# invictus717/MiCo

Measured on AMD Instinct MI355X. Metric: omni-modal samples/sec (ViT-g/14 fwd+bwd), higher is better.
Workload: dtype fp16

## Files before the change

### mico_amd/csrc/attention.hip

```cpp
#include "common.h"
#include <type_traits>

namespace {

constexpr float NEG_BIG = -1.0e30f;

#ifndef MICO_ATTN_PRIO
#define MICO_ATTN_PRIO 0
#endif

#ifdef MICO_ATTN_PHASES
__device__ unsigned long long g_attn_phase[4096 * 8];
#define PH_DECL unsigned long long ph_t = __builtin_readcyclecounter(), ph_acc[8] = {0, 0, 0, 0, 0, 0, 0, 0}
#define PH(slot) do { const unsigned long long n_ = __builtin_readcyclecounter(); ph_acc[slot] += n_ - ph_t; ph_t = n_; } while (0)
#define PH_STORE do { const int wg_ = (blockIdx.z * gridDim.y + blockIdx.y) * gridDim.x + blockIdx.x; \
        if (lane == 0 && wave == 0 && wg_ < 4096) for (int e_ = 0; e_ < 8; ++e_) g_attn_phase[wg_ * 8 + e_] = ph_acc[e_]; } while (0)
#else
#define PH_DECL
#define PH(slot)
#define PH_STORE
#endif

template <int HDP> struct Cfg {
    static constexpr int RS = 256;
// ... 53 lines not shown
}
template <int HDP, int KM = 0>
__device__ __forceinline__ s16x8 lds_row_frag(LDS_AS const char* tile, int r0, int ks, int lane) {
    const int row = r0 + (lane & 15), ch = ks * 4 + (lane >> 4);
    return *(LDS_AS const s16x8*)(tile + row * Cfg<HDP>::RS + ((ch ^ swz_key<KM>(row)) << 4));
}
template <int HDP, int KM = 0>
__device__ __forceinline__ s16x8 lds_tr_frag(LDS_AS const char* tile, int td, int s2, int lane) {
    const int g = lane >> 4, p = lane & 15;
    const int ch = td * 2 + ((p >> 1) & 1), half = (p & 1) * 8;
    const int r_lo = (2 * s2) * 16 + g * 4 + (p >> 2);
    const int col_b = ((ch ^ swz_key<KM>(r_lo)) << 4) + half;
    s16x4 lo = __builtin_amdgcn_ds_read_tr16_b64_v4i16((LDS_AS s16x4*)(tile + r_lo * Cfg<HDP>::RS + col_b));
    s16x4 hi = __builtin_amdgcn_ds_read_tr16_b64_v4i16((LDS_AS s16x4*)(tile + (r_lo + 16) * Cfg<HDP>::RS + col_b));
    s16x8 r;
    r[0] = lo[0]; r[1] = lo[1]; r[2] = lo[2]; r[3] = lo[3];
    r[4] = hi[0]; r[5] = hi[1]; r[6] = hi[2]; r[7] = hi[3];
    return r;
}

__device__ __forceinline__ void lds_dma16(__amdgpu_buffer_rsrc_t rsrc, unsigned lds_dst, unsigned voffset) {
    unsigned keep;
    const unsigned dst = __builtin_amdgcn_readfirstlane(lds_dst);
    asm volatile("s_mov_b32 %0, m0\n\ts_mov_b32 m0, %2\n\ts_nop 0\n\tbuffer_load_dwordx4 %1, %3, 0 offen lds\n\ts_mov_b32 m0, %0"
                 : "=&s"(keep) : "v"(voffset), "s"(dst), "s"(rsrc) : "memory");
}

__device__ __forceinline__ void* uniform_ptr(const void* ptr) {
    const unsigned long long v = (unsigned long long)ptr;
    const unsigned lo = __builtin_amdgcn_readfirstlane((unsigned)v), hi = __builtin_amdgcn_readfirstlane((unsigned)(v >> 32));
    return (void*)(((unsigned long long)hi << 32) | lo);
}

template <typename T>
__device__ __forceinline__ s16x8 pack_pair(const f32x4& a, const f32x4& b) {
    typename T16<T>::v8 v;
    v[0] = (T)a[0]; v[1] = (T)a[1]; v[2] = (T)a[2]; v[3] = (T)a[3];
    v[4] = (T)b[0]; v[5] = (T)b[1]; v[6] = (T)b[2]; v[7] = (T)b[3];
    return __builtin_bit_cast(s16x8, v);
}

__device__ __forceinline__ float group_max(float v) { return xor32_max(xor16_max(v)); }
__device__ __forceinline__ float group_sum(float v) { return xor32_sum(xor16_sum(v)); }

__device__ __forceinline__ float mask_val(const float* mask, int mode, int b, int i, int j, int Sq, int Sk) {
    if (mode == 1) return mask[(int64_t)b * Sk + j];
    if (mode == 2) return mask[((int64_t)b * Sq + i) * Sk + j];
    return 0.f;
}

template <typename T, int HDP, bool DROP, int RB, int NW = 4>
__global__ __launch_bounds__(NW * 64, 2) void attn_fwd_kernel(const T* __restrict__ q, const T* __restrict__ k,
                                                              const T* __restrict__ v, T* __restrict__ o,
                                                              float* __restrict__ lse, const mico_attn_params p) {
    using C = Cfg<HDP>;
    __shared__ __attribute__((aligned(16))) char smem[2 * C::TILE];
    LDS_AS char* kt = (LDS_AS char*)smem;
    LDS_AS char* vt = kt + C::TILE;
    const int tid = threadIdx.x, lane = tid & 63, wave = tid >> 6;
    const bool stager = NW == 4 || tid < 256;
    const int b = blockIdx.z, h = blockIdx.y, q0 = blockIdx.x * (NW * 16 * RB);
    const T* qb = q + (int64_t)b * p.q_bs + h * p.hd;
    const int kvb = p.kv_index ? p.kv_index[b] : (p.kv_batch_mod > 0 ? b % p.kv_batch_mod : b);
    const T* kb = k + (int64_t)kvb * p.k_bs + h * p.hd;
    const T* vb = v + (int64_t)kvb * p.v_bs + h * p.hd;
    const int i0 = q0 + wave * (16 * RB) + (lane & 15);
    const int g = lane >> 4;
    const bool wave_live = q0 + wave * (16 * RB) < p.Sq;

    s16x8 qf[RB][C::KS];
    f32x4 oacc[RB][C::TD];
    float m_run[RB], l_run[RB];
#pragma unroll
    for (int rb = 0; rb < RB; ++rb) {
        row_frags<T, HDP>(qf[rb], qb, p.q_rs, i0 + rb * 16, p.Sq, p.hd, lane);
#pragma unroll
        for (int t = 0; t < C::TD; ++t) oacc[rb][t] = (f32x4){0.f, 0.f, 0.f, 0.f};
        m_run[rb] = NEG_BIG;
        l_run[rb] = 0.f;
    }
    const float sc2 = p.scale * 1.4426950408889634f;

    const int nt = (p.Sk + 63) / 64;
    const TileMap<HDP> tm_a = tile_map<HDP>(p.k_rs, p.hd, tid), tm_b = tile_map<HDP>(p.v_rs, p.hd, tid);
    s16x8 kr[C::NCH], vr[C::NCH];
    if (stager) {
        tile_fetch<T, HDP>(kr, kb, p.k_rs, 0, p.Sk, tm_a);
        tile_fetch<T, HDP>(vr, vb, p.v_rs, 0, p.Sk, tm_b);
    }
    PH_DECL;
    for (int t = 0; t < nt; ++t) {
        __syncthreads();
        PH(0);
        if (stager) {
            tile_commit<HDP>(kr, kt, tm_a);
            tile_commit<HDP>(vr, vt, tm_b);
        }
        PH(1);
        __syncthreads();
        PH(2);
        if (stager && t + 1 < nt) {
            tile_fetch<T, HDP>(kr, kb, p.k_rs, (t + 1) * 64, p.Sk, tm_a);
            tile_fetch<T, HDP>(vr, vb, p.v_rs, (t + 1) * 64, p.Sk, tm_b);
        }
        PH(3);
        const bool edge = (t == nt - 1) && (p.Sk & 63);
        const int ntn = edge ? ((p.Sk - t * 64 + 15) >> 4) : 4;
        f32x4 s[RB][4];
#pragma unroll
        for (int tn = 0; tn < 4; ++tn) {
#pragma unroll
            for (int rb = 0; rb < RB; ++rb) s[rb][tn] = (f32x4){0.f, 0.f, 0.f, 0.f};
            if (tn < ntn && wave_live) {
#pragma unroll
                for (int ks = 0; ks < C::KS; ++ks) {
                    const s16x8 a = lds_row_frag<HDP>(kt, tn * 16, ks, lane);
#pragma unroll
                    for (int rb = 0; rb < RB; ++rb) s[rb][tn] = T16<T>::mfma(a, qf[rb][ks], s[rb][tn]);
                }
            }
        }
        s16x8 pf[RB][2];
        PH(4);
#pragma unroll
        for (int rb = 0; rb < RB; ++rb) {
            const int i = i0 + rb * 16;
            float mloc = NEG_BIG;
            if (!p.mask_mode && !edge) {
#pragma unroll
                for (int tn = 0; tn < 4; ++tn) {
                    s[rb][tn] *= sc2;
                    mloc = fmaxf(fmaxf(mloc, fmaxf(s[rb][tn][0], s[rb][tn][1])), fmaxf(s[rb][tn][2], s[rb][tn][3]));
                }
            } else {
#pragma unroll
                for (int tn = 0; tn < 4; ++tn)
#pragma unroll
                    for (int r = 0; r < 4; ++r) {
                        const int j = t * 64 + tn * 16 + g * 4 + r;
                        float x = s[rb][tn][r] * sc2;
                        if (j < p.Sk) {
                            if (p.mask_mode && i < p.Sq) x += mask_val(p.mask, p.mask_mode, b, i, j, p.Sq, p.Sk) * 1.4426950408889634f;
                        } else {
                            x = NEG_BIG;
                        }
                        s[rb][tn][r] = x;
                        mloc = fmaxf(mloc, x);
                    }
            }
// ... 11 lines not shown
            if (DROP) {
                const unsigned thr = drop_threshold(p.drop_p);
                const float ik = 1.f / (1.f - p.drop_p);
                const unsigned long long rowbase = (((unsigned long long)(b + p.batch0) * p.H + h) * p.Sq + i) * (unsigned long long)p.Sk;
                if ((unsigned long long)(p.B + p.batch0) * p.H * p.Sq * p.Sk <= 0xFFFFFFFFull) {
                    const unsigned h0 = p.drop_seed ^ ((unsigned)p.drop_site * 0x9E3779B9u);
                    const unsigned tb = ((unsigned)rowbase + (unsigned)(t * 64 + g * 4)) * 0x85EBCA6Bu;
#pragma unroll
                    for (int tn = 0; tn < 4; ++tn)
#pragma unroll
                        for (int r = 0; r < 4; ++r)
                            s[rb][tn][r] *= drop_hash_t(h0, tb + (unsigned)(tn * 16 + r) * 0x85EBCA6Bu) >= thr ? ik : 0.f;
                } else {
#pragma unroll
                    for (int tn = 0; tn < 4; ++tn)
#pragma unroll
                        for (int r = 0; r < 4; ++r)
                            s[rb][tn][r] *= drop_mult(p.drop_seed, p.drop_site, rowbase + (t * 64 + tn * 16 + g * 4 + r), thr, ik);
                }
            }
            l_run[rb] = l_run[rb] * alpha + group_sum(lloc);
            m_run[rb] = m_new;
#pragma unroll
            for (int t2 = 0; t2 < C::TD; ++t2) oacc[rb][t2] *= alpha;
            pf[rb][0] = pack_pair<T>(s[rb][0], s[rb][1]);
            pf[rb][1] = pack_pair<T>(s[rb][2], s[rb][3]);
        }
        PH(5);
#pragma unroll
        for (int s2 = 0; s2 < 2; ++s2) {
            if (2 * s2 >= ntn || !wave_live) continue;
#pragma unroll
            for (int td = 0; td < C::TD; ++td) {
                const s16x8 a = lds_tr_frag<HDP>(vt, td, s2, lane);
#pragma unroll
                for (int rb = 0; rb < RB; ++rb) oacc[rb][td] = T16<T>::mfma(a, pf[rb][s2], oacc[rb][td]);
            }
        }
        PH(6);
    }
    PH_STORE;
#pragma unroll
    for (int rb = 0; rb < RB; ++rb) {
        const int i = i0 + rb * 16;
        if (i < p.Sq) {
            const float inv = 1.f / l_run[rb];
            T* ob = o + (int64_t)b * p.o_bs + (int64_t)i * p.o_rs + h * p.hd;
#pragma unroll
            for (int td = 0; td < C::TD; ++td) {
                const int d = td * 16 + g * 4;
                if (d < p.hd)
                    *(s16x4*)(ob + d) = pack4<T>(oacc[rb][td][0] * inv, oacc[rb][td][1] * inv, oacc[rb][td][2] * inv, oacc[rb][td][3] * inv);
            }
            if (g == 0) lse[((int64_t)b * p.H + h) * p.Sq + i] = (m_run[rb] + __log2f(l_run[rb])) * 0.6931471805599453f;
        }
    }
}

constexpr int RES_KR = 288;

template <typename T, int HDP, int RB, int NSUB, bool ALL>
__device__ __forceinline__ void res_tile_step(LDS_AS const char* ktile, LDS_AS const char* vtile, const int key0, const int lo,
                                              const int hi, const int mode, const s16x8 (&qf)[RB][Cfg<HDP>::KS],
                                              f32x4 (&oacc)[RB][Cfg<HDP>::TD], float (&m_run)[RB], float (&l_run)[RB],
                                              const int Sk, const float sc2, const int lane,
                                              const int (&rf)[Cfg<HDP>::KS], const int (&tf)[Cfg<HDP>::TD]) {
    using C = Cfg<HDP>;
    constexpr int NH = (NSUB + 1) / 2;
    const int g = lane >> 4;
    f32x4 s[RB][NH * 2];
    if (ALL) {
        s16x8 an[C::KS];
#pragma unroll
// ... 1529 lines not shown
        }
        if (lane < 24) {
            LDS_AS float* pw = part + wave * 2 * HDP + lane * 4;
#pragma unroll
            for (int e = 0; e < 4; ++e) { pw[e] = dkx[e]; pw[HDP + e] = dvx[e]; }
        }
        asm volatile("s_waitcnt lgkmcnt(0)" ::: "memory");
        __builtin_amdgcn_s_barrier();
        if (tid < 2 * HDP / 4) {
            const int which = tid / (HDP / 4), d = (tid - which * (HDP / 4)) * 4;
            f32x4 acc = {0.f, 0.f, 0.f, 0.f};
            for (int w = 0; w < 8; ++w) {
                LDS_AS const float* prow = part + w * 2 * HDP + which * HDP + d;
                acc[0] += prow[0]; acc[1] += prow[1]; acc[2] += prow[2]; acc[3] += prow[3];
            }
            if (d < p.hd) {
                T* out = (which ? dv + (int64_t)b * p.v_bs + (int64_t)256 * p.v_rs : dk + (int64_t)b * p.k_bs + (int64_t)256 * p.k_rs) + h * p.hd + d;
                *(s16x4*)out = pack4<T>(acc[0], acc[1], acc[2], acc[3]);
            }
        }
    }
}

#endif
struct SqCfg {
    static constexpr int QMAX = 80, QR = 96;
    static constexpr int RS = 128;
    static constexpr int QT = QR * RS;
    static constexpr int KT = 32 * RS, DST = 32 * 256, WAVE = KT + DST;
    static constexpr int STAT = 2 * QR * 4;
    static constexpr int LDS = 2 * QT + STAT + 4 * WAVE;
};

__device__ __forceinline__ int sq_off(int row, int ch) { return row * SqCfg::RS + ((ch ^ ((((row >> 1) & 3) << 1) | ((row >> 3) & 1))) << 4); }
__device__ __forceinline__ s16x8 sq_row_frag(LDS_AS const char* tile, int r0, int ks, int lane) {
    return *(LDS_AS const s16x8*)(tile + sq_off(r0 + (lane & 15), ks * 4 + (lane >> 4)));
}
__device__ __forceinline__ s16x8 sq_tr_frag(LDS_AS const char* tile, int td, int s2, int lane) {
    const int g = lane >> 4, p = lane & 15;
    const int r_lo = (2 * s2) * 16 + g * 4 + (p >> 2);
    const int off = sq_off(r_lo, td * 2 + ((p >> 1) & 1)) + (p & 1) * 8;
    s16x4 lo = __builtin_amdgcn_ds_read_tr16_b64_v4i16((LDS_AS s16x4*)(tile + off));
    s16x4 hi = __builtin_amdgcn_ds_read_tr16_b64_v4i16((LDS_AS s16x4*)(tile + off + 16 * SqCfg::RS));
    s16x8 r;
    r[0] = lo[0]; r[1] = lo[1]; r[2] = lo[2]; r[3] = lo[3];
    r[4] = hi[0]; r[5] = hi[1]; r[6] = hi[2]; r[7] = hi[3];
    return r;
}

template <typename T, bool DROP, int MASK>
__global__ __launch_bounds__(256, 2) void attn_bwd_smallq_kernel(const T* __restrict__ q, const T* __restrict__ k, const T* __restrict__ v,
                                                                 const T* __restrict__ o, const T* __restrict__ d_o, const float* __restrict__ lse,
                                                                 T* __restrict__ dq, T* __restrict__ dk, T* __restrict__ dv, const mico_attn_params p) {
    using S = SqCfg;
    constexpr int HD = 64;
    __shared__ __attribute__((aligned(16))) char smem[S::LDS];
    LDS_AS char* qt = (LDS_AS char*)smem;
    LDS_AS char* dot = qt + S::QT;
    LDS_AS float* lse_t = (LDS_AS float*)(dot + S::QT);
    LDS_AS float* del_t = lse_t + S::QR;
    LDS_AS char* strips = (LDS_AS char*)smem + 2 * S::QT + S::STAT;
    const int tid = threadIdx.x, lane = tid & 63, wave = __builtin_amdgcn_readfirstlane(tid >> 6), g = lane >> 4;
    const int b = blockIdx.y, h = blockIdx.x;
    LDS_AS char* kt = strips + wave * S::WAVE;
    LDS_AS char* dst = kt + S::KT;
    const T* qb = q + (int64_t)b * p.q_bs + h * HD;
    const int kvb = p.kv_batch_mod > 0 ? b % p.kv_batch_mod : b;
    const T* kb = k + (int64_t)kvb * p.k_bs + h * HD;
    const T* vb = v + (int64_t)kvb * p.v_bs + h * HD;
    const T* ob = o + (int64_t)b * p.o_bs + h * HD;
    const T* dob = d_o + (int64_t)b * p.o_bs + h * HD;
    const int64_t stat_base = ((int64_t)b * p.H + h) * p.Sq;
    constexpr float LOG2E = 1.4426950408889634f;
    const float sc2 = p.scale * LOG2E;
    const int nstrips = (p.Sk + 31) >> 5, nrounds = (nstrips + 3) >> 2;

    s16x8 kf[2][2], vf[2][2];
#pragma unroll
    for (int kbk = 0; kbk < 2; ++kbk) {
        row_frags<T, HD>(kf[kbk], kb, p.k_rs, wave * 32 + kbk * 16 + (lane & 15), p.Sk, HD, lane);
        row_frags<T, HD>(vf[kbk], vb, p.v_rs, wave * 32 + kbk * 16 + (lane & 15), p.Sk, HD, lane);
    }
#pragma unroll
    for (int it = 0; it < 3; ++it) {
        const int c = it * 256 + tid, row = c >> 3, ch = c & 7;
        s16x8 qv = {0, 0, 0, 0, 0, 0, 0, 0}, dv8 = qv, ov = qv;
        if (row < p.Sq) {
            qv = *(const s16x8*)(qb + (int64_t)row * p.q_rs + ch * 8);
            dv8 = *(const s16x8*)(dob + (int64_t)row * p.o_rs + ch * 8);
            ov = *(const s16x8*)(ob + (int64_t)row * p.o_rs + ch * 8);
        }
        *(LDS_AS s16x8*)(qt + sq_off(row, ch)) = qv;
        *(LDS_AS s16x8*)(dot + sq_off(row, ch)) = dv8;
        float a[8], c8[8], dl = 0.f;
        unpack8<T>(ov, a);
        unpack8<T>(dv8, c8);
#pragma unroll
        for (int e = 0; e < 8; ++e) dl += a[e] * c8[e];
        dl += __shfl_xor(dl, 1);
        dl += __shfl_xor(dl, 2);
        dl += __shfl_xor(dl, 4);
        if (ch == 0) {
            del_t[row] = dl * p.scale;
            lse_t[row] = row < p.Sq ? lse[stat_base + row] * LOG2E : 0.f;
        }
    }
    __syncthreads();

    f32x4 dqw[4], dq4 = {0.f, 0.f, 0.f, 0.f};
#pragma unroll
    for (int td = 0; td < 4; ++td) dqw[td] = (f32x4){0.f, 0.f, 0.f, 0.f};

    const int nti = (p.Sq + 15) >> 4;
    const unsigned ibase = (unsigned)((((unsigned long long)(b + p.batch0) * p.H + h) * p.Sq) * (unsigned long long)p.Sk);
    const unsigned h0 = p.drop_seed ^ ((unsigned)p.drop_site * 0x9E3779B9u), tstep = (unsigned)p.Sk * 0x85EBCA6Bu;
    const unsigned thr = drop_threshold(p.drop_p);
    const float inv_keep = 1.f / (1.f - p.drop_p);
    const f32x4 zero4 = {0.f, 0.f, 0.f, 0.f};

    for (int rd = 0; rd < nrounds; ++rd) {
        const int k0 = (rd * 4 + wave) * 32;
        s16x8 nkf[2][2], nvf[2][2];
        if (rd + 1 < nrounds) {
#pragma unroll
            for (int kbk = 0; kbk < 2; ++kbk) {
                row_frags<T, HD>(nkf[kbk], kb, p.k_rs, k0 + 128 + kbk * 16 + (lane & 15), p.Sk, HD, lane);
                row_frags<T, HD>(nvf[kbk], vb, p.v_rs, k0 + 128 + kbk * 16 + (lane & 15), p.Sk, HD, lane);
            }
        }
        if (k0 < p.Sk) {
#pragma unroll
            for (int kbk = 0; kbk < 2; ++kbk)
#pragma unroll
                for (int ks = 0; ks < 2; ++ks) *(LDS_AS s16x8*)(kt + sq_off(kbk * 16 + (lane & 15), ks * 4 + g)) = kf[kbk][ks];
#pragma unroll
            for (int kbk = 0; kbk < 2; ++kbk) {
                __builtin_amdgcn_sched_barrier(0);
                const int j = k0 + kbk * 16 + (lane & 15);
                const bool jv = j < p.Sk;
                const int jc = jv ? j : p.Sk - 1;
                T* const dkb = dk + (int64_t)b * p.k_bs + (int64_t)jc * p.k_rs + h * HD;
                T* const dvb = dv + (int64_t)b * p.v_bs + (int64_t)jc * p.v_rs + h * HD;
                s16x4 okd[4], ovd[4];
                if (MASK == 0 && p.dkv_accumulate == 1) {
#pragma unroll
                    for (int td = 0; td < 4; ++td) {
                        okd[td] = *(const s16x4*)(dkb + td * 16 + g * 4);
                        ovd[td] = *(const s16x4*)(dvb + td * 16 + g * 4);
                    }
                }
                float mk1 = 0.f;
                if (MASK == 1) mk1 = p.mask[(int64_t)b * p.Sk + jc] * LOG2E;
                f32x4 s[5], dp[5];
#pragma unroll
                for (int ti = 0; ti < 5; ++ti) {
                    s[ti] = zero4;
                    dp[ti] = zero4;
                    if (ti < nti) {
#pragma unroll
                        for (int ks = 0; ks < 2; ++ks) {
                            s[ti] = T16<T>::mfma(sq_row_frag(qt, ti * 16, ks, lane), kf[kbk][ks], s[ti]);
                            dp[ti] = T16<T>::mfma(sq_row_frag(dot, ti * 16, ks, lane), vf[kbk][ks], dp[ti]);
                        }
                    }
                }
                const unsigned tq = (ibase + (unsigned)j + (unsigned)(4 * g) * (unsigned)p.Sk) * 0x85EBCA6Bu;
                f32x4 pr[5];
#pragma unroll
                for (int ti = 0; ti < 5; ++ti) {
                    const f32x4 lv = *(LDS_AS const f32x4*)(lse_t + ti * 16 + g * 4);
                    const f32x4 dv4 = *(LDS_AS const f32x4*)(del_t + ti * 16 + g * 4);
#pragma unroll
                    for (int r = 0; r < 4; ++r) {
                        const int i = ti * 16 + g * 4 + r;
                        const bool ok = jv && i < p.Sq;
                        float x = s[ti][r] * sc2;
                        if (MASK == 1) x += mk1;
                        if (MASK == 2) x += p.mask[((int64_t)b * p.Sq + (i < p.Sq ? i : p.Sq - 1)) * p.Sk + jc] * LOG2E;
                        float pv = __builtin_amdgcn_exp2f(x - lv[r]);
                        float dm = 1.f;
                        if (DROP) dm = drop_hash_t(h0, tq + (unsigned)(ti * 16 + r) * tstep) >= thr ? inv_keep : 0.f;
                        const float ds = pv * fmaf(dp[ti][r] * dm, p.scale, -dv4[r]);
                        pv *= dm;
                        pr[ti][r] = ok ? pv : 0.f;
                        s[ti][r] = ok ? ds : 0.f;
                    }
                    const int row = kbk * 16 + (lane & 15), ch = ti * 2 + (g >> 1);
                    *(LDS_AS s16x4*)(dst + row * 256 + ((ch ^ swz_key<0>(row)) << 4) + (g & 1) * 8) = pack4<T>(s[ti][0], s[ti][1], s[ti][2], s[ti][3]);
                }
                f32x4 dva[4], dka[4];
#pragma unroll
                for (int td = 0; td < 4; ++td) {
                    dva[td] = zero4;
                    dka[td] = zero4;
                }
#pragma unroll
                for (int s2 = 0; s2 < 3; ++s2) {
                    if (2 * s2 >= nti) continue;
                    const s16x8 pf = pack_pair<T>(pr[2 * s2], s2 < 2 ? pr[2 * s2 + 1] : zero4);
                    const s16x8 df = pack_pair<T>(s[2 * s2], s2 < 2 ? s[2 * s2 + 1] : zero4);
#pragma unroll
                    for (int td = 0; td < 4; ++td) {
                        dva[td] = T16<T>::mfma(sq_tr_frag(dot, td, s2, lane), pf, dva[td]);
                        dka[td] = T16<T>::mfma(sq_tr_frag(qt, td, s2, lane), df, dka[td]);
                    }
                }
                if (jv) {
#pragma unroll
                    for (int td = 0; td < 4; ++td) {
                        const int d = td * 16 + g * 4;
                        if (p.dkv_accumulate) {
                            if (MASK == 0 && p.dkv_accumulate == 1) {
                                dka[td] += unpack4<T>(okd[td]);
                                dva[td] += unpack4<T>(ovd[td]);
                            } else {
                                dka[td] += unpack4<T>(*(const s16x4*)(dkb + d));
                                dva[td] += unpack4<T>(*(const s16x4*)(dvb + d));
                            }
                        }
                        *(s16x4*)(dkb + d) = pack4<T>(dka[td][0], dka[td][1], dka[td][2], dka[td][3]);
                        *(s16x4*)(dvb + d) = pack4<T>(dva[td][0], dva[td][1], dva[td][2], dva[td][3]);
                    }
                }
            }
        }
        __syncthreads();
        __builtin_amdgcn_sched_barrier(0);
#pragma unroll
        for (int st = 0; st < 4; ++st) {
            if ((rd * 4 + st) * 32 >= p.Sk) continue;
            LDS_AS const char* skt = strips + st * S::WAVE;
            LDS_AS const char* sdst = skt + S::KT;
            if (wave < nti) {
                const s16x8 dsf = lds_tr_frag<64, 0>(sdst, wave, 0, lane);
#pragma unroll
                for (int td = 0; td < 4; ++td) dqw[td] = T16<T>::mfma(sq_tr_frag(skt, td, 0, lane), dsf, dqw[td]);
            }
            if (nti == 5) dq4 = T16<T>::mfma(sq_tr_frag(skt, wave, 0, lane), lds_tr_frag<64, 0>(sdst, 4, 0, lane), dq4);
        }
        __syncthreads();
#pragma unroll
        for (int kbk = 0; kbk < 2; ++kbk)
#pragma unroll
            for (int ks = 0; ks < 2; ++ks) {
                kf[kbk][ks] = nkf[kbk][ks];
                vf[kbk][ks] = nvf[kbk][ks];
            }
    }

    {
        const int i = wave * 16 + (lane & 15);
        if (i < p.Sq) {
            T* dqb = dq + (int64_t)b * p.q_bs + (int64_t)i * p.q_rs + h * HD;
#pragma unroll
            for (int td = 0; td < 4; ++td) *(s16x4*)(dqb + td * 16 + g * 4) = pack4<T>(dqw[td][0], dqw[td][1], dqw[td][2], dqw[td][3]);
        }
        const int i4 = 64 + (lane & 15);
        if (i4 < p.Sq)
            *(s16x4*)(dq + (int64_t)b * p.q_bs + (int64_t)i4 * p.q_rs + h * HD + wave * 16 + g * 4) = pack4<T>(dq4[0], dq4[1], dq4[2], dq4[3]);
    }
}

template <int HDP> struct OpCfg {
    using C = Cfg<HDP>;
    static constexpr int NST = 3;
    static constexpr int QT = 32 * C::RS;
    static constexpr int STAGE = 2 * QT;
    static constexpr int KROWS = 272;
    static constexpr int KT = KROWS * C::RS;
    static constexpr int DSK = 32 * 64;
    static constexpr int DSB = 8 * DSK;
// ... 515 lines not shown
    } while (0)

#ifdef MICO_ATTN_PHASES
extern "C" int mico_debug_attn_phases(unsigned long long* out, int n) {
    return (int)hipMemcpyFromSymbol(out, HIP_SYMBOL(g_attn_phase), sizeof(unsigned long long) * n);
}
#endif

extern "C" int mico_attn_fwd(const void* q, const void* k, const void* v, void* o, float* lse, const mico_attn_params* p,
                             int dtype, void* stream) {
    MICO_CHECK(dtype_ok(dtype) && q && k && v && o && lse, "mico_attn_fwd: bad args");
    int rc = check_params(p, "mico_attn_fwd");
    if (rc) return rc;
    const dim3 block(256);
    hipStream_t st = (hipStream_t)stream;
    static const bool no_res = getenv("MICO_ATTN_NORES") != nullptr;
    if (!no_res && p->kv_batch_mod == 0 && !p->kv_index && p->mask_mode == 0 && p->drop_p <= 0.f && p->hd <= 96 && p->k_rs == p->v_rs && p->Sq > 128 && p->Sk <= 272 && p->Sq <= 256 + ResCfg<96>::NXMAX) {
        static const int n_cu = [] { int dev = 0, n = 256; (void)hipGetDevice(&dev); (void)hipDeviceGetAttribute(&n, hipDeviceAttributeMultiprocessorCount, dev); return n > 0 ? n : 256; }();
        const int nitems = p->B * p->H;
        const dim3 grid(nitems < n_cu ? nitems : n_cu);
        DISPATCH_T16(dtype, {
            if (p->hd <= 64) MICO_LAUNCH((attn_fwd_res_kernel<T, 64>), grid, dim3(512), 0, st, (const T*)q, (const T*)k, (const T*)v, (T*)o, lse, *p);
            else MICO_LAUNCH((attn_fwd_res_kernel<T, 96>), grid, dim3(512), 0, st, (const T*)q, (const T*)k, (const T*)v, (T*)o, lse, *p);
        });
        MICO_LAUNCH_CHECK();
        return MICO_OK;
    }
    const bool two = p->Sq > 64 && p->drop_p <= 0.f;
    static const bool no_five = getenv("MICO_ATTN_NOFIVE") != nullptr;
    const bool five = !two && !no_five && p->drop_p > 0.f && p->Sq > 64 && p->Sq <= 80 && p->hd <= 64;
    const int qpw = two ? 128 : (five ? 80 : 64);
    const dim3 grid((p->Sq + qpw - 1) / qpw, p->H, p->B);
#define ATTN_FWD_LAUNCH(DROP, RB) MICO_LAUNCH((attn_fwd_kernel<T, HDP, DROP, RB>), grid, block, 0, st, (const T*)q, (const T*)k, (const T*)v, (T*)o, lse, *p)
    if (five) {
        DISPATCH_T16(dtype, MICO_LAUNCH((attn_fwd_kernel<T, 64, true, 1, 5>), grid, dim3(320), 0, st, (const T*)q, (const T*)k, (const T*)v, (T*)o, lse, *p));
        MICO_LAUNCH_CHECK();
        return MICO_OK;
    }
    DISPATCH_T16(dtype, ATTN_DISPATCH_HD(p->hd, {
        if (two) ATTN_FWD_LAUNCH(false, 2);
        else if (p->drop_p > 0.f) ATTN_FWD_LAUNCH(true, 1);
        else ATTN_FWD_LAUNCH(false, 1);
    }));
#undef ATTN_FWD_LAUNCH
    MICO_LAUNCH_CHECK();
    return MICO_OK;
}

extern "C" int mico_attn_bwd(const void* q, const void* k, const void* v, const void* o, const void* d_o, const float* lse,
                             void* dq, void* dk, void* dv, float* delta, const mico_attn_params* p, int dtype,
                             void* stream) {
    MICO_CHECK(dtype_ok(dtype) && q && k && v && o && d_o && lse && dq && dk && dv && delta, "mico_attn_bwd: bad args");
    int rc = check_params(p, "mico_attn_bwd");
    if (rc) return rc;
    MICO_CHECK(!p->kv_index, "mico_attn_bwd: kv_index is an inference feature of mico_attn_fwd (dK / dV of an indexed K/V memory would need a scatter-add)");
    hipStream_t st = (hipStream_t)stream;
    const dim3 block(256);
    static const bool no_smallq = getenv("MICO_ATTN_NOSMALLQ") != nullptr;
    if (!no_smallq && p->hd == 64 && p->Sq <= SqCfg::QMAX && (p->drop_p <= 0.f || (unsigned long long)(p->B + p->batch0) * p->H * p->Sq * p->Sk <= 0xFFFFFFFFull)) {
        const dim3 grid(p->H, p->B);
        static const bool no_pf = getenv("MICO_SMALLQ_NOPF") != nullptr;
        mico_attn_params pp = *p;
        pp.dkv_accumulate = p->dkv_accumulate ? (no_pf ? 2 : 1) : 0;
#define SQ_LAUNCH(DROP, MASK) MICO_LAUNCH((attn_bwd_smallq_kernel<T, DROP, MASK>), grid, block, 0, st, (const T*)q, (const T*)k, (const T*)v, (const T*)o, (const T*)d_o, lse, (T*)dq, (T*)dk, (T*)dv, pp)
        DISPATCH_T16(dtype, {
            if (p->drop_p > 0.f) { if (p->mask_mode == 0) SQ_LAUNCH(true, 0); else if (p->mask_mode == 1) SQ_LAUNCH(true, 1); else SQ_LAUNCH(true, 2); }
            else { if (p->mask_mode == 0) SQ_LAUNCH(false, 0); else if (p->mask_mode == 1) SQ_LAUNCH(false, 1); else SQ_LAUNCH(false, 2); }
        });
#undef SQ_LAUNCH
        MICO_LAUNCH_CHECK();
        return MICO_OK;
    }
    MICO_CHECK(!p->dkv_accumulate, "mico_attn_bwd: dkv_accumulate is implemented by the short-query kernel only (Sq <= %d at hd 64)", SqCfg::QMAX);
    const dim3 gq((p->Sq + 63) / 64, p->H, p->B), gk((p->Sk + 63) / 64, p->H, p->B);
    static const bool no_res = getenv("MICO_ATTN_NORES") != nullptr;
    const bool res = !no_res && p->kv_batch_mod == 0 && p->mask_mode == 0 && p->drop_p <= 0.f && p->hd <= 96 && p->k_rs == p->v_rs && p->Sq > 128 && p->Sk <= 272 &&
                     p->Sq <= 256 + ResCfg<96>::NXMAX;
    static const bool no_onepass = getenv("MICO_ATTN_NOONEPASS") != nullptr;
    if (res && !no_onepass && p->Sk <= 257) {
        static const int n_cu1 = [] { int dev = 0, n = 256; (void)hipGetDevice(&dev); (void)hipDeviceGetAttribute(&n, hipDeviceAttributeMultiprocessorCount, dev); return n > 0 ? n : 256; }();
        const int nitems = p->B * p->H;
        const dim3 grid(nitems < n_cu1 ? nitems : n_cu1);
#define OP_LAUNCH(HDP, KMODE) MICO_LAUNCH((attn_bwd_onepass_kernel<T, HDP, KMODE>), grid, dim3(512), 0, st, (const T*)q, (const T*)k, (const T*)v, (const T*)o, (const T*)d_o, lse, (T*)dq, (T*)dk, (T*)dv, *p)
        DISPATCH_T16(dtype, {
            if (p->hd <= 64) { if (p->Sk == 257) OP_LAUNCH(64, 2); else if (p->Sk == 256) OP_LAUNCH(64, 1); else OP_LAUNCH(64, 0); }
            else { if (p->Sk == 257) OP_LAUNCH(96, 2); else if (p->Sk == 256) OP_LAUNCH(96, 1); else OP_LAUNCH(96, 0); }
        });
#undef OP_LAUNCH
        MICO_LAUNCH_CHECK();
        return MICO_OK;
    }
    if (res) {
        static const int n_cu = [] { int dev = 0, n = 256; (void)hipGetDevice(&dev); (void)hipDeviceGetAttribute(&n, hipDeviceAttributeMultiprocessorCount, dev); return n > 0 ? n : 256; }();
        const int nitems = p->B * p->H;
        const dim3 grid(nitems < n_cu ? nitems : n_cu);
        DISPATCH_T16(dtype, {
            if (p->hd <= 64) MICO_LAUNCH((attn_bwd_dq_res_kernel<T, 64>), grid, dim3(512), 0, st, (const T*)q, (const T*)k, (const T*)v, (const T*)o, (const T*)d_o, lse, (T*)dq, delta, *p);
            else MICO_LAUNCH((attn_bwd_dq_res_kernel<T, 96>), grid, dim3(512), 0, st, (const T*)q, (const T*)k, (const T*)v, (const T*)o, (const T*)d_o, lse, (T*)dq, delta, *p);
        });
    } else
    DISPATCH_T16(dtype, ATTN_DISPATCH_HD(p->hd, { if (p->drop_p > 0.f) MICO_LAUNCH((attn_bwd_dq_kernel<T, HDP, true>), gq, block, 0, st, (const T*)q, (const T*)k, (const T*)v, (const T*)o, (const T*)d_o, lse, (T*)dq, delta, *p); else MICO_LAUNCH((attn_bwd_dq_kernel<T, HDP, false>), gq, block, 0, st, (const T*)q, (const T*)k, (const T*)v, (const T*)o, (const T*)d_o, lse, (T*)dq, delta, *p); }));
// ... 26 lines not shown
```

### mico_amd/csrc/common.h

```cpp
#pragma once
#include <hip/hip_runtime.h>
#include <stdint.h>
#include "../../include/mico_hip.h"

typedef _Float16 f16;
typedef __bf16 bf16;
typedef float f32x4 __attribute__((ext_vector_type(4)));
typedef float f32x2 __attribute__((ext_vector_type(2)));
typedef _Float16 f16x8 __attribute__((ext_vector_type(8)));
typedef _Float16 f16x4 __attribute__((ext_vector_type(4)));
typedef __bf16 bf16x8 __attribute__((ext_vector_type(8)));
typedef __bf16 bf16x4 __attribute__((ext_vector_type(4)));
typedef short s16x8 __attribute__((ext_vector_type(8)));
typedef short s16x4 __attribute__((ext_vector_type(4)));
typedef unsigned int u32x4 __attribute__((ext_vector_type(4)));
typedef unsigned int u32x2 __attribute__((ext_vector_type(2)));

#define LDS_AS __attribute__((address_space(3)))

extern thread_local char g_mico_err[256];
int mico_set_err(int code, const char* fmt, ...);

#define MICO_CHECK(cond, ...)                         \
    do {                                              \
// ... 118 lines not shown
    e2 = (f32x2){__builtin_amdgcn_exp2f(w[0]), __builtin_amdgcn_exp2f(w[1])};
    const f32x2 y = poly * t * e2;
    const f32x2 y2 = (f32x2){2.0f, 2.0f} - y;
    const f32x2 ope = {z[0] >= 0.f ? y2[0] : y[0], z[1] >= 0.f ? y2[1] : y[1]};
    cdf = ope * 0.5f;
}
__device__ __forceinline__ f32x4 gelu4(const f32x4 x) {
    f32x2 c0, c1, e0, e1;
    gelu_terms2((f32x2){x[0], x[1]}, c0, e0);
    gelu_terms2((f32x2){x[2], x[3]}, c1, e1);
    const f32x2 g0 = (f32x2){x[0], x[1]} * c0, g1 = (f32x2){x[2], x[3]} * c1;
    return (f32x4){g0[0], g0[1], g1[0], g1[1]};
}
__device__ __forceinline__ f32x4 gelu_pair4(const f32x4 x, f32x4& deriv) {
    f32x2 c0, c1, e0, e1;
    const f32x2 x0 = {x[0], x[1]}, x1 = {x[2], x[3]};
    gelu_terms2(x0, c0, e0);
    gelu_terms2(x1, c1, e1);
    const f32x2 d0 = __builtin_elementwise_fma(x0 * 0.39894228040143268f, e0, c0), d1 = __builtin_elementwise_fma(x1 * 0.39894228040143268f, e1, c1);
    const f32x2 g0 = x0 * c0, g1 = x1 * c1;
    deriv = (f32x4){d0[0], d0[1], d1[0], d1[1]};
    return (f32x4){g0[0], g0[1], g1[0], g1[1]};
}

__device__ __forceinline__ unsigned drop_hash(unsigned seed, int site, unsigned long long idx) {
    unsigned h = seed ^ ((unsigned)site * 0x9E3779B9u);
    h ^= (unsigned)idx * 0x85EBCA6Bu;
    h = ((h << 13) | (h >> 19)) * 5u + 0xE6546B64u;
    h ^= (unsigned)(idx >> 32) * 0xC2B2AE35u;
    h = ((h << 13) | (h >> 19)) * 5u + 0xE6546B64u;
    h ^= h >> 16; h *= 0x85EBCA6Bu; h ^= h >> 13; h *= 0xC2B2AE35u; h ^= h >> 16;
    return h >> 8;
}
__device__ __forceinline__ unsigned drop_hash_t(unsigned h0, unsigned t) {
    unsigned h = h0 ^ t;
    h = ((h << 13) | (h >> 19)) * 5u + 0xE6546B64u;
    h = ((h << 13) | (h >> 19)) * 5u + 0xE6546B64u;
    h ^= h >> 16; h *= 0x85EBCA6Bu; h ^= h >> 13; h *= 0xC2B2AE35u; h ^= h >> 16;
    return h >> 8;
}
__device__ __forceinline__ float drop_mult(unsigned seed, int site, unsigned long long idx, unsigned thr, float inv_keep) {
    return drop_hash(seed, site, idx) >= thr ? inv_keep : 0.f;
}
__host__ __device__ __forceinline__ unsigned drop_threshold(float p) { return (unsigned)(p * 16777216.f); }

#define MICO_XLANE(NAME, INSN, OP)                                                  \
    __device__ __forceinline__ float NAME(float v) {                                 \
        float a = v, b = v;                                                          \
        asm volatile("s_nop 1\n\t" INSN " %0, %1" : "+v"(a), "+v"(b));               \
        return OP;                                                                   \
    }
MICO_XLANE(xor16_sum, "v_permlane16_swap_b32", a + b)
MICO_XLANE(xor32_sum, "v_permlane32_swap_b32", a + b)
MICO_XLANE(xor16_max, "v_permlane16_swap_b32", fmaxf(a, b))
MICO_XLANE(xor32_max, "v_permlane32_swap_b32", fmaxf(a, b))
#undef MICO_XLANE
#define MICO_DPP_F32(v, ctrl) __builtin_bit_cast(float, __builtin_amdgcn_update_dpp(0, __builtin_bit_cast(int, v), ctrl, 0xf, 0xf, true))
__device__ __forceinline__ float row16_sum(float v) {
    v += MICO_DPP_F32(v, 0xb1);
    v += MICO_DPP_F32(v, 0x4e);
    v += MICO_DPP_F32(v, 0x124);
    v += MICO_DPP_F32(v, 0x128);
    return v;
}
__device__ __forceinline__ float row16_max(float v) {
    v = fmaxf(v, MICO_DPP_F32(v, 0xb1));
    v = fmaxf(v, MICO_DPP_F32(v, 0x4e));
    v = fmaxf(v, MICO_DPP_F32(v, 0x124));
    v = fmaxf(v, MICO_DPP_F32(v, 0x128));
    return v;
// ... 19 lines not shown
```

Baseline: 44.25.

## Stage forward attention K/V tiles via triple-buffered LDS DMA; reswizzle small-Q backward strips

The forward attention kernel gains a DMA variant for head dim 64. It loads K/V tiles straight into a three-deep LDS ring using buffer_load ... lds, replacing register-staged fetch-and-commit with two syncthreads per tile by a single waitcnt plus barrier. The small-Q backward kernel switches to a new XOR swizzle for the Q/dO strips and the dS tile, with precomputed lane offsets meant to cut LDS bank conflicts; the old layout stays behind an env var. A multiply-by-5 in the dropout hash is rewritten as shift-plus-add. The new path uses much more LDS per block, which may lower occupancy, and depends on the vmcnt ordering being correct.

```diff
diff --git a/mico_amd/csrc/attention.hip b/mico_amd/csrc/attention.hip
--- a/mico_amd/csrc/attention.hip
+++ b/mico_amd/csrc/attention.hip
@@ -109,6 +109,15 @@
     return (void*)(((unsigned long long)hi << 32) | lo);
 }
 
+template <bool OLD = false> __device__ __forceinline__ int sq_off(int row, int ch);
+template <bool OLD = false> __device__ __forceinline__ s16x8 sq_row_frag(LDS_AS const char* tile, int r0, int ks, int lane);
+template <bool OLD = false> __device__ __forceinline__ s16x8 sq_tr_frag(LDS_AS const char* tile, int td, int s2, int lane);
+
+struct FwdDma {
+    static constexpr int TILE = 64 * 128, NBUF = 3, PIECES = 4;
+    static constexpr int LDS = NBUF * 2 * TILE;
+};
+
 template <typename T>
 __device__ __forceinline__ s16x8 pack_pair(const f32x4& a, const f32x4& b) {
     typename T16<T>::v8 v;
@@ -126,14 +135,15 @@
     return 0.f;
 }
 
-template <typename T, int HDP, bool DROP, int RB, int NW = 4>
+template <typename T, int HDP, bool DROP, int RB, int NW = 4, bool DMA = false>
 __global__ __launch_bounds__(NW * 64, 2) void attn_fwd_kernel(const T* __restrict__ q, const T* __restrict__ k,
                                                               const T* __restrict__ v, T* __restrict__ o,
                                                               float* __restrict__ lse, const mico_attn_params p) {
     using C = Cfg<HDP>;
-    __shared__ __attribute__((aligned(16))) char smem[2 * C::TILE];
+    static_assert(!DMA || HDP == 64, "the LDS-DMA staged image is the compact 64-wide one");
+    __shared__ __attribute__((aligned(1024))) char smem[DMA ? FwdDma::LDS : 2 * C::TILE];
     LDS_AS char* kt = (LDS_AS char*)smem;
-    LDS_AS char* vt = kt + C::TILE;
+    LDS_AS char* vt = kt + (DMA ? FwdDma::TILE : C::TILE);
     const int tid = threadIdx.x, lane = tid & 63, wave = tid >> 6;
     const bool stager = NW == 4 || tid < 256;
     const int b = blockIdx.z, h = blockIdx.y, q0 = blockIdx.x * (NW * 16 * RB);
@@ -159,14 +169,55 @@
     const float sc2 = p.scale * 1.4426950408889634f;
 
     const int nt = (p.Sk + 63) / 64;
-    const TileMap<HDP> tm_a = tile_map<HDP>(p.k_rs, p.hd, tid), tm_b = tile_map<HDP>(p.v_rs, p.hd, tid);
+    TileMap<HDP> tm_a, tm_b;
     s16x8 kr[C::NCH], vr[C::NCH];
-    if (stager) {
+    const __amdgpu_buffer_rsrc_t rk = __builtin_amdgcn_make_buffer_rsrc(uniform_ptr(kb), 0, __builtin_amdgcn_readfirstlane((int)(((int64_t)(p.Sk - 1) * p.k_rs + p.hd) * 2)), 0x00020000);
+    const __amdgpu_buffer_rsrc_t rv = __builtin_amdgcn_make_buffer_rsrc(uniform_ptr(vb), 0, __builtin_amdgcn_readfirstlane((int)(((int64_t)(p.Sk - 1) * p.v_rs + p.hd) * 2)), 0x00020000);
+    const unsigned lds0 = (unsigned)(uintptr_t)kt;
+    unsigned ko0 = 0, vo0 = 0, kstep = 0, vstep = 0;
+    if constexpr (DMA) {
+        const int sch = (lane & 7) ^ ((lane >> 3) & 7), srow = (wave & 3) * 8 + ((lane >> 3) & 7);
+        const unsigned dead = sch * 8 < p.hd ? 0u : 0x80000000u;
+        ko0 = ((unsigned)(srow * (int)p.k_rs + sch * 8) * 2u) | dead;
+        vo0 = ((unsigned)(srow * (int)p.v_rs + sch * 8) * 2u) | dead;
+        kstep = (unsigned)p.k_rs * 64u;
+        vstep = (unsigned)p.v_rs * 64u;
+    } else {
+        tm_a = tile_map<HDP>(p.k_rs, p.hd, tid);
+        tm_b = tile_map<HDP>(p.v_rs, p.hd, tid);
+    }
+    auto dma_tile = [&](int tt, int buf) {
+        const unsigned dstk = lds0 + (unsigned)(buf * 2 * FwdDma::TILE + (wave & 3) * 1024);
+        const unsigned tk = ko0 + (unsigned)tt * 2u * kstep, tv = vo0 + (unsigned)tt * 2u * vstep;
+        lds_dma16(rk, dstk, tk);
+        lds_dma16(rk, dstk + 4096, tk + kstep);
+        lds_dma16(rv, dstk + FwdDma::TILE, tv);
+        lds_dma16(rv, dstk + FwdDma::TILE + 4096, tv + vstep);
+    };
+    if constexpr (DMA) {
+        if (stager) {
+            dma_tile(0, 0);
+            dma_tile(1, 1);
+        }
+    } else if (stager) {
         tile_fetch<T, HDP>(kr, kb, p.k_rs, 0, p.Sk, tm_a);
         tile_fetch<T, HDP>(vr, vb, p.v_rs, 0, p.Sk, tm_b);
     }
+    int cur = 0;
     PH_DECL;
     for (int t = 0; t < nt; ++t) {
+        if constexpr (DMA) {
+            asm volatile("s_waitcnt vmcnt(4)" ::: "memory");
+            __builtin_amdgcn_s_barrier();
+            __builtin_amdgcn_sched_barrier(0);
+            PH(0);
+            if (stager) dma_tile(t + 2, cur == 0 ? 2 : cur - 1);
+            __builtin_amdgcn_sched_barrier(0);
+            kt = (LDS_AS char*)smem + cur * (2 * FwdDma::TILE);
+            vt = kt + FwdDma::TILE;
+            cur = cur == 2 ? 0 : cur + 1;
+            PH(3);
+        } else {
         __syncthreads();
         PH(0);
         if (stager) {
@@ -181,6 +232,7 @@
             tile_fetch<T, HDP>(vr, vb, p.v_rs, (t + 1) * 64, p.Sk, tm_b);
         }
         PH(3);
+        }
         const bool edge = (t == nt - 1) && (p.Sk & 63);
         const int ntn = edge ? ((p.Sk - t * 64 + 15) >> 4) : 4;
         f32x4 s[RB][4];
@@ -191,7 +243,7 @@
             if (tn < ntn && wave_live) {
 #pragma unroll
                 for (int ks = 0; ks < C::KS; ++ks) {
-                    const s16x8 a = lds_row_frag<HDP>(kt, tn * 16, ks, lane);
+                    const s16x8 a = DMA ? sq_row_frag(kt, tn * 16, ks, lane) : lds_row_frag<HDP>(kt, tn * 16, ks, lane);
 #pragma unroll
                     for (int rb = 0; rb < RB; ++rb) s[rb][tn] = T16<T>::mfma(a, qf[rb][ks], s[rb][tn]);
                 }
@@ -269,13 +321,14 @@
             if (2 * s2 >= ntn || !wave_live) continue;
 #pragma unroll
             for (int td = 0; td < C::TD; ++td) {
-                const s16x8 a = lds_tr_frag<HDP>(vt, td, s2, lane);
+                const s16x8 a = DMA ? sq_tr_frag(vt, td, s2, lane) : lds_tr_frag<HDP>(vt, td, s2, lane);
 #pragma unroll
                 for (int rb = 0; rb < RB; ++rb) oacc[rb][td] = T16<T>::mfma(a, pf[rb][s2], oacc[rb][td]);
             }
         }
         PH(6);
     }
+    if constexpr (DMA) asm volatile("s_waitcnt vmcnt(0)" ::: "memory");
     PH_STORE;
 #pragma unroll
     for (int rb = 0; rb < RB; ++rb) {
@@ -1871,14 +1924,16 @@
     static constexpr int LDS = 2 * QT + STAT + 4 * WAVE;
 };
 
-__device__ __forceinline__ int sq_off(int row, int ch) { return row * SqCfg::RS + ((ch ^ ((((row >> 1) & 3) << 1) | ((row >> 3) & 1))) << 4); }
-__device__ __forceinline__ s16x8 sq_row_frag(LDS_AS const char* tile, int r0, int ks, int lane) {
-    return *(LDS_AS const s16x8*)(tile + sq_off(r0 + (lane & 15), ks * 4 + (lane >> 4)));
-}
-__device__ __forceinline__ s16x8 sq_tr_frag(LDS_AS const char* tile, int td, int s2, int lane) {
+template <bool OLD> __device__ __forceinline__ int sq_off(int row, int ch) {
+    return row * SqCfg::RS + ((ch ^ (OLD ? ((((row >> 1) & 3) << 1) | ((row >> 3) & 1)) : (row & 7))) << 4);
+}
+template <bool OLD> __device__ __forceinline__ s16x8 sq_row_frag(LDS_AS const char* tile, int r0, int ks, int lane) {
+    return *(LDS_AS const s16x8*)(tile + sq_off<OLD>(r0 + (lane & 15), ks * 4 + (lane >> 4)));
+}
+template <bool OLD> __device__ __forceinline__ s16x8 sq_tr_frag(LDS_AS const char* tile, int td, int s2, int lane) {
     const int g = lane >> 4, p = lane & 15;
     const int r_lo = (2 * s2) * 16 + g * 4 + (p >> 2);
-    const int off = sq_off(r_lo, td * 2 + ((p >> 1) & 1)) + (p & 1) * 8;
+    const int off = sq_off<OLD>(r_lo, td * 2 + ((p >> 1) & 1)) + (p & 1) * 8;
     s16x4 lo = __builtin_amdgcn_ds_read_tr16_b64_v4i16((LDS_AS s16x4*)(tile + off));
     s16x4 hi = __builtin_amdgcn_ds_read_tr16_b64_v4i16((LDS_AS s16x4*)(tile + off + 16 * SqCfg::RS));
     s16x8 r;
@@ -1887,7 +1942,21 @@
     return r;
 }
 
-template <typename T, bool DROP, int MASK>
+template <bool OLD> __device__ __forceinline__ int dst_off(int row, int ch, int half) {
+    return OLD ? row * 256 + ((ch ^ swz_key<0>(row)) << 4) + half * 8
+               : row * 256 + ((ch ^ (((row & 7) << 1) | ((row >> 2) & 1))) << 4) + ((half ^ (row >> 3)) & 1) * 8;
+}
+__device__ __forceinline__ s16x8 dst_tr_frag(LDS_AS const char* tile, int lane_off, int td) {
+    const int off = lane_off ^ (td << 5);
+    s16x4 lo = __builtin_amdgcn_ds_read_tr16_b64_v4i16((LDS_AS s16x4*)(tile + off));
+    s16x4 hi = __builtin_amdgcn_ds_read_tr16_b64_v4i16((LDS_AS s16x4*)(tile + off + 16 * 256));
+    s16x8 r;
+    r[0] = lo[0]; r[1] = lo[1]; r[2] = lo[2]; r[3] = lo[3];
+    r[4] = hi[0]; r[5] = hi[1]; r[6] = hi[2]; r[7] = hi[3];
+    return r;
+}
+
+template <typename T, bool DROP, int MASK, bool OLDSTRIP = false>
 __global__ __launch_bounds__(256, 2) void attn_bwd_smallq_kernel(const T* __restrict__ q, const T* __restrict__ k, const T* __restrict__ v,
                                                                  const T* __restrict__ o, const T* __restrict__ d_o, const float* __restrict__ lse,
                                                                  T* __restrict__ dq, T* __restrict__ dk, T* __restrict__ dv, const mico_attn_params p) {
@@ -1929,8 +1998,8 @@
             dv8 = *(const s16x8*)(dob + (int64_t)row * p.o_rs + ch * 8);
             ov = *(const s16x8*)(ob + (int64_t)row * p.o_rs + ch * 8);
         }
-        *(LDS_AS s16x8*)(qt + sq_off(row, ch)) = qv;
-        *(LDS_AS s16x8*)(dot + sq_off(row, ch)) = dv8;
+        *(LDS_AS s16x8*)(qt + sq_off<OLDSTRIP>(row, ch)) = qv;
+        *(LDS_AS s16x8*)(dot + sq_off<OLDSTRIP>(row, ch)) = dv8;
         float a[8], c8[8], dl = 0.f;
         unpack8<T>(ov, a);
         unpack8<T>(dv8, c8);
@@ -1956,6 +2025,8 @@
     const unsigned thr = drop_threshold(p.drop_p);
     const float inv_keep = 1.f / (1.f - p.drop_p);
     const f32x4 zero4 = {0.f, 0.f, 0.f, 0.f};
+    const int dsw = dst_off<OLDSTRIP>(lane & 15, g >> 1, g & 1);
+    const int dsr = dst_off<OLDSTRIP>(g * 4 + ((lane & 15) >> 2), (lane >> 1) & 1, lane & 1);
 
     for (int rd = 0; rd < nrounds; ++rd) {
         const int k0 = (rd * 4 + wave) * 32;
@@ -1971,7 +2042,7 @@
 #pragma unroll
             for (int kbk = 0; kbk < 2; ++kbk)
 #pragma unroll
-                for (int ks = 0; ks < 2; ++ks) *(LDS_AS s16x8*)(kt + sq_off(kbk * 16 + (lane & 15), ks * 4 + g)) = kf[kbk][ks];
+                for (int ks = 0; ks < 2; ++ks) *(LDS_AS s16x8*)(kt + sq_off<OLDSTRIP>(kbk * 16 + (lane & 15), ks * 4 + g)) = kf[kbk][ks];
 #pragma unroll
             for (int kbk = 0; kbk < 2; ++kbk) {
                 __builtin_amdgcn_sched_barrier(0);
@@ -1998,8 +2069,8 @@
                     if (ti < nti) {
 #pragma unroll
                         for (int ks = 0; ks < 2; ++ks) {
-                            s[ti] = T16<T>::mfma(sq_row_frag(qt, ti * 16, ks, lane), kf[kbk][ks], s[ti]);
-                            dp[ti] = T16<T>::mfma(sq_row_frag(dot, ti * 16, ks, lane), vf[kbk][ks], dp[ti]);
+                            s[ti] = T16<T>::mfma(sq_row_frag<OLDSTRIP>(qt, ti * 16, ks, lane), kf[kbk][ks], s[ti]);
+                            dp[ti] = T16<T>::mfma(sq_row_frag<OLDSTRIP>(dot, ti * 16, ks, lane), vf[kbk][ks], dp[ti]);
                         }
                     }
                 }
@@ -2024,8 +2095,7 @@
                         pr[ti][r] = ok ? pv : 0.f;
                         s[ti][r] = ok ? ds : 0.f;
                     }
-                    const int row = kbk * 16 + (lane & 15), ch = ti * 2 + (g >> 1);
-                    *(LDS_AS s16x4*)(dst + row * 256 + ((ch ^ swz_key<0>(row)) << 4) + (g & 1) * 8) = pack4<T>(s[ti][0], s[ti][1], s[ti][2], s[ti][3]);
+                    *(LDS_AS s16x4*)(dst + ((dsw ^ (ti << 5)) + kbk * 16 * 256)) = pack4<T>(s[ti][0], s[ti][1], s[ti][2], s[ti][3]);
                 }
                 f32x4 dva[4], dka[4];
 #pragma unroll
@@ -2040,8 +2110,8 @@
                     const s16x8 df = pack_pair<T>(s[2 * s2], s2 < 2 ? s[2 * s2 + 1] : zero4);
 #pragma unroll
                     for (int td = 0; td < 4; ++td) {
-                        dva[td] = T16<T>::mfma(sq_tr_frag(dot, td, s2, lane), pf, dva[td]);
-                        dka[td] = T16<T>::mfma(sq_tr_frag(qt, td, s2, lane), df, dka[td]);
+                        dva[td] = T16<T>::mfma(sq_tr_frag<OLDSTRIP>(dot, td, s2, lane), pf, dva[td]);
+                        dka[td] = T16<T>::mfma(sq_tr_frag<OLDSTRIP>(qt, td, s2, lane), df, dka[td]);
                     }
                 }
                 if (jv) {
@@ -2071,11 +2141,11 @@
             LDS_AS const char* skt = strips + st * S::WAVE;
             LDS_AS const char* sdst = skt + S::KT;
             if (wave < nti) {
-                const s16x8 dsf = lds_tr_frag<64, 0>(sdst, wave, 0, lane);
-#pragma unroll
-                for (int td = 0; td < 4; ++td) dqw[td] = T16<T>::mfma(sq_tr_frag(skt, td, 0, lane), dsf, dqw[td]);
-            }
-            if (nti == 5) dq4 = T16<T>::mfma(sq_tr_frag(skt, wave, 0, lane), lds_tr_frag<64, 0>(sdst, 4, 0, lane), dq4);
+                const s16x8 dsf = dst_tr_frag(sdst, dsr, wave);
+#pragma unroll
+                for (int td = 0; td < 4; ++td) dqw[td] = T16<T>::mfma(sq_tr_frag<OLDSTRIP>(skt, td, 0, lane), dsf, dqw[td]);
+            }
+            if (nti == 5) dq4 = T16<T>::mfma(sq_tr_frag<OLDSTRIP>(skt, wave, 0, lane), dst_tr_frag(sdst, dsr, 4), dq4);
         }
         __syncthreads();
 #pragma unroll
@@ -2657,6 +2727,22 @@
     const int qpw = two ? 128 : (five ? 80 : 64);
     const dim3 grid((p->Sq + qpw - 1) / qpw, p->H, p->B);
 #define ATTN_FWD_LAUNCH(DROP, RB) MICO_LAUNCH((attn_fwd_kernel<T, HDP, DROP, RB>), grid, block, 0, st, (const T*)q, (const T*)k, (const T*)v, (T*)o, lse, *p)
+    static const bool no_dma = getenv("MICO_ATTN_NODMA") != nullptr;
+    const int64_t nt64 = (p->Sk + 63) / 64, rs_max = p->k_rs > p->v_rs ? p->k_rs : p->v_rs;
+    const bool dma = !no_dma && !two && p->hd <= 64 && (p->hd & 7) == 0 && nt64 > 1 && (((uintptr_t)k | (uintptr_t)v) & 15) == 0 &&
+                     p->k_rs > 0 && p->v_rs > 0 && p->k_bs >= 0 && p->v_bs >= 0 && ((p->k_rs | p->v_rs | p->k_bs | p->v_bs) & 7) == 0 &&
+                     (nt64 + 2) * 64 * rs_max * 2 + 4096 < (1ll << 31);
+#define ATTN_FWD_DMA_LAUNCH(DROP, NW) MICO_LAUNCH((attn_fwd_kernel<T, 64, DROP, 1, NW, true>), grid, dim3(NW * 64), 0, st, (const T*)q, (const T*)k, (const T*)v, (T*)o, lse, *p)
+    if (dma) {
+        DISPATCH_T16(dtype, {
+            if (five) ATTN_FWD_DMA_LAUNCH(true, 5);
+            else if (p->drop_p > 0.f) ATTN_FWD_DMA_LAUNCH(true, 4);
+            else ATTN_FWD_DMA_LAUNCH(false, 4);
+        });
+        MICO_LAUNCH_CHECK();
+        return MICO_OK;
+    }
+#undef ATTN_FWD_DMA_LAUNCH
     if (five) {
         DISPATCH_T16(dtype, MICO_LAUNCH((attn_fwd_kernel<T, 64, true, 1, 5>), grid, dim3(320), 0, st, (const T*)q, (const T*)k, (const T*)v, (T*)o, lse, *p));
         MICO_LAUNCH_CHECK();
@@ -2687,11 +2773,14 @@
         static const bool no_pf = getenv("MICO_SMALLQ_NOPF") != nullptr;
         mico_attn_params pp = *p;
         pp.dkv_accumulate = p->dkv_accumulate ? (no_pf ? 2 : 1) : 0;
-#define SQ_LAUNCH(DROP, MASK) MICO_LAUNCH((attn_bwd_smallq_kernel<T, DROP, MASK>), grid, block, 0, st, (const T*)q, (const T*)k, (const T*)v, (const T*)o, (const T*)d_o, lse, (T*)dq, (T*)dk, (T*)dv, pp)
+        static const bool old_strip = getenv("MICO_SMALLQ_OLDSTRIP") != nullptr;
+#define SQ_LAUNCH_(DROP, MASK, OLD) MICO_LAUNCH((attn_bwd_smallq_kernel<T, DROP, MASK, OLD>), grid, block, 0, st, (const T*)q, (const T*)k, (const T*)v, (const T*)o, (const T*)d_o, lse, (T*)dq, (T*)dk, (T*)dv, pp)
+#define SQ_LAUNCH(DROP, MASK) do { if (old_strip) SQ_LAUNCH_(DROP, MASK, true); else SQ_LAUNCH_(DROP, MASK, false); } while (0)
         DISPATCH_T16(dtype, {
             if (p->drop_p > 0.f) { if (p->mask_mode == 0) SQ_LAUNCH(true, 0); else if (p->mask_mode == 1) SQ_LAUNCH(true, 1); else SQ_LAUNCH(true, 2); }
             else { if (p->mask_mode == 0) SQ_LAUNCH(false, 0); else if (p->mask_mode == 1) SQ_LAUNCH(false, 1); else SQ_LAUNCH(false, 2); }
         });
+#undef SQ_LAUNCH_
 #undef SQ_LAUNCH
         MICO_LAUNCH_CHECK();
         return MICO_OK;
diff --git a/mico_amd/csrc/common.h b/mico_amd/csrc/common.h
--- a/mico_amd/csrc/common.h
+++ b/mico_amd/csrc/common.h
@@ -174,10 +174,14 @@
     h ^= h >> 16; h *= 0x85EBCA6Bu; h ^= h >> 13; h *= 0xC2B2AE35u; h ^= h >> 16;
     return h >> 8;
 }
+__device__ __forceinline__ unsigned drop_round(unsigned h) {
+    h = (h << 13) | (h >> 19);
+    unsigned h4 = h << 2;
+    asm("" : "+v"(h4));
+    return h4 + h + 0xE6546B64u;
+}
 __device__ __forceinline__ unsigned drop_hash_t(unsigned h0, unsigned t) {
-    unsigned h = h0 ^ t;
-    h = ((h << 13) | (h >> 19)) * 5u + 0xE6546B64u;
-    h = ((h << 13) | (h >> 19)) * 5u + 0xE6546B64u;
+    unsigned h = drop_round(drop_round(h0 ^ t));
     h ^= h >> 16; h *= 0x85EBCA6Bu; h ^= h >> 13; h *= 0xC2B2AE35u; h ^= h >> 16;
     return h >> 8;
 }
```

Result: no change. 44.25 (median of 2 runs) (+0.0%).
